# microsoft/Spartan2

Hardware: AMD Instinct MI355X
Metric: sha256_spartan prove(): R1CS constraints/sec (prove wall-clock in ms_per_step) (higher is better)
Workload: dtype u256 modular integer (8 x u32 Montgomery limbs; T256 scalar/base fields)

## Files before the change

### spartan2_amd/csrc/capi_core.hip

```cpp
#include <atomic>
#include <chrono>
#include <cstdlib>
#include <cstdio>
#include <cstring>

#include "core.hpp"
#include "walk_pool.hpp"
#include "kernels_poly.hpp"

namespace sp {
static thread_local std::string g_err;
static thread_local sp_wait_hook g_wait_hook = nullptr;
static thread_local void* g_wait_user = nullptr;
void set_error(const std::string& m) { g_err = m; }
static std::atomic<int> g_live_contexts{0};
int live_contexts() { return g_live_contexts.load(std::memory_order_relaxed); }
void relax() {
  if (g_wait_hook) g_wait_hook(g_wait_user);
  else __builtin_ia32_pause();
}
void slow_note(const char* site, long spins) {
  static const bool on = getenv("SPARTAN_SLOWPATH_LOG") != nullptr;
  if (on) fprintf(stderr, "[slow path] %s after %ld polls\n", site, spins);
}
// ... 546 lines not shown
}
static bool fold_stage2_enabled() {
  static const bool on = [] {
    const char* e = getenv("SPARTAN_FOLD_STAGE2");
    return e && e[0] == '1';
  }();
  return on;
}
static spk::LazyOut lazy_out(sp_ctx* c, spk::lazy9_t* lp, size_t nparts, int gl, const fe_t* eq_out, unsigned seq) {
  spk::LazyOut lo(lp);
  const size_t ngroups = nparts >> gl;
  size_t b2 = (ngroups + 63) / 64;
  if (b2 < 1) b2 = 1;
  if (b2 > (size_t)spk::HOST_SUM_MAX_BLOCKS) b2 = spk::HOST_SUM_MAX_BLOCKS;
  lo.eq_out = eq_out;
  lo.mapped = c->d_pinned;
  lo.seq = seq;
  lo.nslots = (unsigned)b2;
  lo.gl = gl;
  static const unsigned fold_slots = [] {
    const char* e = getenv("SPARTAN_FOLD_SLOTS");
    const int v = e ? atoi(e) : spk::HOST_SUM_MAX_BLOCKS;
    return (unsigned)(v < 1 ? 1 : (v > spk::HOST_SUM_MAX_BLOCKS ? spk::HOST_SUM_MAX_BLOCKS : v));
  }();
  size_t fs = fold_slots;
  while (fs > 1 && (fs > ngroups || ngroups % fs)) fs >>= 1;
  const bool even = ngroups > 0 && ((size_t)ngroups << gl) == nparts && ngroups % fs == 0 && (gl == 0 || nparts % 2 == 0);
  if (fold_stage2_enabled() && even && c->d_fold_tickets) {
    lo.tickets = c->d_fold_tickets;
    lo.nslots = (unsigned)fs;
    lo.per_slot = (unsigned)(nparts / fs);
  }
  return lo;
}
static void sum_lazy_launch(sp_ctx* c, const spk::LazyOut& lo, size_t nparts) {
  const int gl = lo.gl;
  const unsigned seq = lo.seq;
  const fe_t* eq_out = lo.eq_out;
  c->pending_slots = lo.nslots;
  if (lo.tickets) return;
  const uint32_t* P = reinterpret_cast<const uint32_t*>(lo.P);
  const dim3 g(lo.nslots), b(64);
  const bool vec_ok = nparts % 8 == 0;
  if (vec_ok && gl == 0) hipLaunchKernelGGL((spk::k_sum_partials_lazy<0>), g, b, 0, c->stream, P, nparts, gl, eq_out, c->d_pinned, seq);
  else if (vec_ok && gl == 1) hipLaunchKernelGGL((spk::k_sum_partials_lazy<1>), g, b, 0, c->stream, P, nparts, gl, eq_out, c->d_pinned, seq);
  else if (vec_ok && gl == 2) hipLaunchKernelGGL((spk::k_sum_partials_lazy<2>), g, b, 0, c->stream, P, nparts, gl, eq_out, c->d_pinned, seq);
  else if (vec_ok && gl == 3) hipLaunchKernelGGL((spk::k_sum_partials_lazy<3>), g, b, 0, c->stream, P, nparts, gl, eq_out, c->d_pinned, seq);
  else hipLaunchKernelGGL((spk::k_sum_partials_lazy<-1>), g, b, 0, c->stream, P, nparts, gl, eq_out, c->d_pinned, seq);
}
static int wait_slot(sp_ctx* c, const fe_t* slot, unsigned want, int nvals, fe_t* v, bool resident, long* spins) {
  volatile const unsigned* fl = reinterpret_cast<volatile const unsigned*>(slot + 3);
  while (*fl != want) {
    if (++*spins > 400000) {
      sp::slow_note("wait_slot", *spins);
      if (resident) {
        const auto t0 = std::chrono::steady_clock::now();
        while (*fl != want) {
          if (std::chrono::steady_clock::now() - t0 > std::chrono::seconds(12)) return fail(SP_ERR_INTERNAL, "sum-check tail kernel did not deliver a round result");
          sp::relax();
        }
        break;
      }
      SP_HIP(sp::stream_sync(c->stream));
      if (*fl != want) return fail(SP_ERR_INTERNAL, "evaluation kernel did not deliver its block sums");
    }
    sp::relax();
// ... 336 lines not shown
      c->h_mail[spk::MAIL_LINE_WORDS * l + 12] = v;
    }
    if (c->mail_dev) __builtin_ia32_sfence();
  };
  set_all(1);
  sp::stream_sync(c->stream);
  set_all(0);
  *reinterpret_cast<volatile uint32_t*>(c->h_pinned + spk::TAIL_ERR_ELEM) = 0;
}
struct AheadGuard {
  sp_ctx* c;
  bool armed = false;
  explicit AheadGuard(sp_ctx* ctx) : c(ctx) {}
  ~AheadGuard() {
    if (armed) tail_abort(c);
  }
};
static spk::MailRef mail_ref(sp_ctx* c, bool ahead, unsigned answers) {
  spk::MailRef m;
  m.mail = ahead ? c->d_mail : nullptr;
  m.mirror = c->d_mail_mirror;
  m.mapped = c->d_pinned;
  m.answers = answers;
  m.gated = nullptr;
  return m;
}
static spk::MailRef gate_launch(sp_ctx* c, unsigned answers) {
  fe_t* slot = c->d_gate + (answers & (spk::MAIL_RING - 1));
  hipLaunchKernelGGL(spk::k_mail_gate, dim3(1), dim3(64), 0, c->stream, mail_ref(c, true, answers), slot);
  spk::MailRef m = mail_ref(c, false, answers);
  m.gated = slot;
  return m;
}
static bool gate_ok(sp_ctx* c) {
  static const bool off = [] {
    const char* e = getenv("SPARTAN_GATE");
    return e && e[0] == '0';
  }();
  return c->mail_dev && !off;
}
static bool launch_ahead_ok(sp_ctx* c, size_t table_len) {
  return c->mail_dev && table_len <= ((size_t)1 << 19);
}
static unsigned tail_blocks(size_t len, bool cubic = false) {
  const size_t q = len / 2, wq = cubic ? spk::TAIL_WIDE_Q_CUBIC : spk::TAIL_WIDE_Q;
  if (q <= wq) return 1u;
  const size_t nb = q / wq;
  return (unsigned)(cubic && nb == 2 * (size_t)spk::HOST_SUM_MAX_BLOCKS ? nb / 2 : nb);
}
static std::atomic<int> g_tail_resident{0};
static int tail_block_budget() {
  static const int v = [] {
    const char* e = getenv("SPARTAN_TAIL_BUDGET");
    const int b = e ? atoi(e) : 64;
    return b < 0 ? 0 : b;
  }();
  return v;
}
struct TailLease {
  int n = 0;
  bool take(unsigned blocks) {
    if (blocks <= 1) return true;
    if (g_tail_resident.fetch_add((int)blocks) + (int)blocks > tail_block_budget()) {
      g_tail_resident.fetch_sub((int)blocks);
      return false;
    }
// ... 386 lines not shown
    eq_in = d_pr + spk::eq_level_offset((int)(ell - 1));
    sbits = 63;
    mode = 0;
  }
  const unsigned seq = next_seq(c);
  const dim3 g((unsigned)blocks), b(256);
  c->timed("eval_cubic", 128ull * half, [&] {
    if (mode == 0) hipLaunchKernelGGL((spk::k_eval_cubic<0, false, true>), g, b, 0, c->stream, A->d, B->d, (const fe_t*)nullptr, half, eq_in, eq_out, sbits, d_part, c->d_pinned, seq);
    else if (mode == 1) hipLaunchKernelGGL((spk::k_eval_cubic<1, false, true>), g, b, 0, c->stream, A->d, B->d, (const fe_t*)nullptr, half, eq_in, eq_out, sbits, d_part, c->d_pinned, seq);
    else hipLaunchKernelGGL((spk::k_eval_cubic<2, false, true>), g, b, 0, c->stream, A->d, B->d, (const fe_t*)nullptr, half, eq_in, eq_out, sbits, d_part, c->d_pinned, seq);
  });
  fe_t sums[2];
  if ((rc = reduce_partials(c, blocks, 2, sums))) return rc;
  const fe_t tinf = sums[1], one = fe_one<S>(), tau = taus[0];
  const fe_t eq0 = fe_sub<S>(one, tau), slope = fe_sub<S>(tau, eq0), eqm1 = fe_sub<S>(eq0, slope);
  const fe_t s_0 = fe_zero(), s_1 = fe_zero();
  const fe_t s_leading = fe_mul<S>(slope, tinf);
  const fe_t s_m1 = fe_mul<S>(eqm1, fe_dbl<S>(tinf));
  const fe_t halfc = two_inv();
  const fe_t c1 = fe_sub<S>(fe_mul<S>(fe_sub<S>(s_1, s_m1), halfc), s_leading);
  const fe_t c2 = fe_sub<S>(fe_mul<S>(fe_add<S>(s_1, s_m1), halfc), s_0);
  const fe_t inner_2 = fe_add<S>(c2, fe_dbl<S>(s_leading));
  const fe_t eval_2 = fe_add<S>(s_0, fe_dbl<S>(fe_add<S>(c1, fe_dbl<S>(inner_2))));
  const fe_t c3_3 = fe_add<S>(fe_dbl<S>(s_leading), s_leading);
  const fe_t inner_3 = fe_add<S>(c2, c3_3);
  const fe_t mid_3 = fe_add<S>(fe_add<S>(c1, fe_dbl<S>(inner_3)), inner_3);
  const fe_t eval_3 = fe_add<S>(fe_add<S>(s_0, fe_dbl<S>(mid_3)), mid_3);
  store_fe(out, s_0);
  store_fe(out + 4, eval_2);
  store_fe(out + 8, eval_3);
  return SP_OK;
}

static bool table_dense(const sp_table* t) { return sp::eff_lo(t) == t->len / 2 && sp::eff_hi(t) == t->len / 2; }

static int quad_impl(sp_ctx* c, uint64_t claim_io[4], size_t rounds, sp_table* A, sp_table* B, sp_transcript* tr, sp_reduce_hook reduce, void* reduce_user,
                     sp_challenge_hook observe, void* observe_user, uint64_t* out_cpolys, uint64_t* out_r, uint64_t out_final[8], size_t run_rounds = 0);
int sp_sumcheck_quad(sp_ctx* c, const uint64_t claim_[4], size_t rounds, sp_table* A, sp_table* B, sp_transcript* tr, uint64_t* out_cpolys,
                     uint64_t* out_r, uint64_t out_final[8]) {
  uint64_t claim_io[4];
  memcpy(claim_io, claim_, 32);
  return quad_impl(c, claim_io, rounds, A, B, tr, nullptr, nullptr, sp::pcs_ahead_wants(c, rounds) ? &sp::pcs_ahead_on_challenge : nullptr, c, out_cpolys, out_r, out_final);
}
int sp_sumcheck_quad_observed(sp_ctx* c, const uint64_t claim_[4], size_t rounds, sp_table* A, sp_table* B, sp_transcript* tr, sp_challenge_hook observe,
                              void* user, uint64_t* out_cpolys, uint64_t* out_r, uint64_t out_final[8]) {
  uint64_t claim_io[4];
  memcpy(claim_io, claim_, 32);
  return quad_impl(c, claim_io, rounds, A, B, tr, nullptr, nullptr, observe, user, out_cpolys, out_r, out_final);
}
int sp_sumcheck_quad_sharded(sp_ctx* c, uint64_t claim_io[4], size_t rounds, sp_table* A, sp_table* B, sp_transcript* tr, sp_reduce_hook reduce, void* reduce_user,
                             uint64_t* out_cpolys, uint64_t* out_r, uint64_t out_final[8]) {
  return quad_impl(c, claim_io, rounds, A, B, tr, reduce, reduce_user, nullptr, nullptr, out_cpolys, out_r, out_final);
}

int sp_sumcheck_quad_sharded_observed(sp_ctx* c, uint64_t claim_io[4], size_t rounds, sp_table* A, sp_table* B, sp_transcript* tr, sp_reduce_hook reduce,
                                      void* reduce_user, sp_challenge_hook observe, void* observe_user, uint64_t* out_cpolys, uint64_t* out_r, uint64_t out_final[8]) {
  return quad_impl(c, claim_io, rounds, A, B, tr, reduce, reduce_user, observe, observe_user, out_cpolys, out_r, out_final);
}

int sp_sumcheck_quad_sharded_partial(sp_ctx* c, uint64_t claim_io[4], size_t rounds, size_t run_rounds, sp_table* A, sp_table* B, sp_transcript* tr,
                                     sp_reduce_hook reduce, void* reduce_user, sp_challenge_hook observe, void* observe_user, uint64_t* out_cpolys, uint64_t* out_r) {
  if (run_rounds == 0 || run_rounds >= rounds) return fail(SP_ERR_INVALID_INPUT_LENGTH, "prove_quad (partial): 0 < run_rounds < rounds");
  uint64_t unused[8];
  return quad_impl(c, claim_io, rounds, A, B, tr, reduce, reduce_user, observe, observe_user, out_cpolys, out_r, unused, run_rounds);
}

// ... 97 lines not shown
      have_sums = true;
      return 1;
    }
    if (sparse_stream) {
      const size_t q = A->len / 4;
      const unsigned seq = next_seq(c);
      const spk::LazyOut lp = lazy_out(c, reinterpret_cast<spk::lazy9_t*>(c->d_scratch), q / 256, 2, nullptr, seq);
      c->timed("bind_stream_quad_sparse", 64ull * (A->len / 2) * 2, [&] {
        hipLaunchKernelGGL(spk::k_bind_eval_quad_stream_sparse, dim3((unsigned)(q / 256)), dim3(256), 0, c->stream, A->d, B->d, q, rv, sp::eff_hi(A), sp::eff_hi(B), lp,
                           mref);
      });
      sum_lazy_launch(c, lp, q / 256);
      sp::after_bind(A);
      sp::after_bind(B);
      have_sums = true;
      return 1;
    }
    if (ahead) return 0;
    sp_table* tabs[2] = {A, B};
    have_sums = false;
    int rc2 = launch_bind(c, tabs, 2, rv);
    return rc2 ? rc2 : 1;
  };
  for (size_t round = 0; round < rounds; ++round) {
    const size_t half = A->len / 2, len_now = A->len;
    const double tr0 = round_trace() ? now_us() : 0;
    fe_t sums[2] = {fe_zero(), fe_zero()};
    bool waiting = have_sums;
    if (!have_sums && !host_mode) {
      size_t len = sp::eff_pairs(A);
      if (sp::eff_pairs(B) < len) len = sp::eff_pairs(B);
      if (half < len) len = half;
      if (len >= STREAM_MIN_Q && len % 1024 == 0) {
        const unsigned seq = next_seq(c);
        const size_t hi_max = sp::eff_hi(A) > sp::eff_hi(B) ? sp::eff_hi(A) : sp::eff_hi(B);
        const bool lowhi = hi_max <= len / 2;
        const size_t blocks = len / (256 * (size_t)4);
        const spk::LazyOut lp = lazy_out(c, reinterpret_cast<spk::lazy9_t*>(c->d_scratch), blocks, 2, nullptr, seq);
        c->timed("eval_quad", 64ull * len + 32ull * ((sp::eff_hi(A) < len ? sp::eff_hi(A) : len) + (sp::eff_hi(B) < len ? sp::eff_hi(B) : len)), [&] {
          if (lowhi)
            hipLaunchKernelGGL((spk::k_eval_quad_stream_lowhi<4>), dim3((unsigned)blocks), dim3(256), 0, c->stream, A->d, B->d, half, sp::eff_hi(A), sp::eff_hi(B), lp);
          else
            hipLaunchKernelGGL((spk::k_eval_quad_stream<4>), dim3((unsigned)blocks), dim3(256), 0, c->stream, A->d, B->d, half, sp::eff_hi(A), sp::eff_hi(B), lp);
        });
        sum_lazy_launch(c, lp, blocks);
        waiting = true;
      } else if (len > 0) {
        size_t blocks = (len + chunk - 1) / chunk;
        c->timed("eval_quad", 64ull * len + 32ull * ((sp::eff_hi(A) < len ? sp::eff_hi(A) : len) + (sp::eff_hi(B) < len ? sp::eff_hi(B) : len)),
                 [&] { hipLaunchKernelGGL(spk::k_eval_quad, dim3((unsigned)blocks), dim3(256), 0, c->stream, A->d, B->d, half, len, sp::eff_hi(A), sp::eff_hi(B), c->d_scratch, c->d_pinned, next_seq(c)); });
        reduce_partials_launch(c, blocks, 2);
        waiting = true;
      }
    }
    const unsigned wait_seq = c->result_seq, wait_slots = c->pending_slots;
    const bool wait_resident = in_tail;
    if (wait_resident && !host_mode && spk::tail_hand_over(len_now, tail_hand_n(false))) {
      hA.resize(2 * len_now);
      if ((rc = wait_hand_over(c, wait_seq, (int)(2 * len_now), hA.data()))) return rc;
      hB = hA.data() + len_now;
      host_mode = true;
      hand_seq = wait_seq;
    }
    if (host_mode) {
      host_quad_eval(hA.data(), hB, half, sums);
      waiting = false;
    }
    if (!host_mode && wait_resident && spk::tail_double(false, len_now, tail_hand_n(false))) {
      fe_t S8[8];
// ... 1243 lines not shown
```

### spartan2_amd/csrc/kernels_poly.hpp

```cpp
#pragma once
#include "device_utils.hpp"

namespace spk {

constexpr int RESULT_FLAG_ELEM = 7;
__device__ __forceinline__ void publish_result(fe_t* result, unsigned seq) {
  __threadfence_system();
  __hip_atomic_store(reinterpret_cast<unsigned*>(result + RESULT_FLAG_ELEM), seq, __ATOMIC_RELEASE, __HIP_MEMORY_SCOPE_SYSTEM);
}

constexpr int HOST_SUM_MAX_BLOCKS = 64;
constexpr int SLOT_BASE_ELEM = 64;
struct slot_chk {
  unsigned a, b;
};
constexpr unsigned SLOT_CHK_K = 0x9E3779B1u;
__host__ __device__ __forceinline__ void slot_chk_add(slot_chk& c, const fe_t& v, int k) {
  unsigned plain = 0, ramp = 0;
#pragma unroll
  for (int i = 0; i < 8; ++i) {
    plain += v.v[i];
    ramp += (unsigned)i * v.v[i];
  }
  c.a += plain;
  c.b += (unsigned)(8 * k + 1) * plain + ramp;
}
__device__ __forceinline__ void slot_store_elem(fe_t* dst, const fe_t& v) { *dst = v; }
__device__ __forceinline__ void slot_store_tag(fe_t* slot, unsigned seq, const slot_chk& c) {
  const unsigned long long hi = ((unsigned long long)seq << 32) | (seq * SLOT_CHK_K + c.b);
  const unsigned long long lo = ((unsigned long long)(seq + c.a) << 32) | seq;
  __hip_atomic_store(reinterpret_cast<unsigned long long*>(&slot[3].v[2]), hi, __ATOMIC_RELAXED, __HIP_MEMORY_SCOPE_SYSTEM);
  __hip_atomic_store(reinterpret_cast<unsigned long long*>(&slot[3].v[0]), lo, __ATOMIC_RELAXED, __HIP_MEMORY_SCOPE_SYSTEM);
}
template <int NACC>
// ... 141 lines not shown
      if (lane == 0) {
        unsigned* e = reinterpret_cast<unsigned*>(mapped + TAIL_ERR_ELEM);
        e[1] = want;
        e[2] = blockIdx.x;
        e[3] = gridDim.x;
        __hip_atomic_store(e, 1u, __ATOMIC_RELEASE, __HIP_MEMORY_SCOPE_SYSTEM);
      }
    }
    if (lane == 0) ok = good;
  }
  __syncthreads();
  return ok != 0;
}
__device__ __forceinline__ fe_t gated_challenge(const fe_t* p) {
  typedef const __attribute__((address_space(4))) uint32_t* const_words;
  const_words q = (const_words)(uintptr_t)p;
  fe_t r;
#pragma unroll
  for (int i = 0; i < 8; ++i) r.v[i] = q[i];
  return r;
}
__device__ __forceinline__ fe_t challenge_or(const MailRef& m, const fe_t& r_arg) {
  if (m.gated) return gated_challenge(m.gated);
  if (!m.mail) return r_arg;
  __shared__ fe_t r_sh;
  mail_wait(m.mail, m.mirror, m.mapped, m.answers, &r_sh);
  return r_sh;
}

__global__ void __launch_bounds__(64) k_mail_gate(MailRef m, fe_t* __restrict__ out) {
  __shared__ fe_t r_sh;
  mail_wait(m.mail, m.mirror, m.mapped, m.answers, &r_sh);
  if (threadIdx.x < 8) out->v[threadIdx.x] = r_sh.v[threadIdx.x];
}

constexpr int BIND_MAX_TABLES = 8;
struct BindArgs {
  fe_t* z[BIND_MAX_TABLES];
  unsigned long long n[BIND_MAX_TABLES];
  unsigned long long lo[BIND_MAX_TABLES];
  unsigned long long hi[BIND_MAX_TABLES];
  fe_t r;
  fe_t one_minus_r;
};
__global__ void __launch_bounds__(256) k_bind_top(BindArgs a) {
  const int t = blockIdx.y;
  fe_t* __restrict__ Z = a.z[t];
  const unsigned long long n = a.n[t], lo = a.lo[t], hi = a.hi[t];
  const unsigned long long eff = lo > hi ? lo : hi;
  const unsigned long long both = lo < hi ? lo : hi;
  for (unsigned long long i = (unsigned long long)blockIdx.x * blockDim.x + threadIdx.x; i < eff; i += (unsigned long long)gridDim.x * blockDim.x) {
    fe_t out;
    if (i < both) {
      fe_t lo_v = Z[i], hi_v = Z[n + i];
      out = fe_add<S>(lo_v, fe_mul<S>(a.r, fe_sub<S>(hi_v, lo_v)));
    } else if (i < lo) {
      out = fe_mul<S>(Z[i], a.one_minus_r);
    } else {
      out = fe_mul<S>(a.r, Z[n + i]);
    }
    Z[i] = out;
  }
}

__host__ __device__ __forceinline__ size_t eq_level_offset(int k) { return ((size_t)1 << k) - 1; }
constexpr int EQ_LDS_ENTRIES = 1024;
// ... 158 lines not shown
      const fe_t eo = eq_out[base >> s];
      acc[0] = fe_mul<S>(acc[0], eo);
      acc[1] = fe_mul<S>(acc[1], eo);
    }
    emit_partials<2>(acc, partials, single_out, seq);
  }
}
__global__ void __launch_bounds__(256) k_bind_eval_quad(fe_t* __restrict__ A, fe_t* __restrict__ B, size_t q, fe_t r_arg, fe_t* __restrict__ partials,
                                                        fe_t* __restrict__ single_out, unsigned seq, MailRef mref) {
  __shared__ fe_t smem[2 * 4];
  const size_t id = (size_t)blockIdx.x * blockDim.x + threadIdx.x;
  const bool live = id < q;
  const size_t ld = live ? id : 0;
  const fe_t la0 = A[ld], la1 = A[ld + q], la2 = A[ld + 2 * q], la3 = A[ld + 3 * q];
  const fe_t lb0 = B[ld], lb1 = B[ld + q], lb2 = B[ld + 2 * q], lb3 = B[ld + 3 * q];
  const fe_t r = challenge_or(mref, r_arg);
  fe_t acc[2] = {fe_zero(), fe_zero()};
  if (live) {
    const fe_t a0 = bind1(la0, la2, r), a1 = bind1(la1, la3, r);
    const fe_t b0 = bind1(lb0, lb2, r), b1 = bind1(lb1, lb3, r);
    A[id] = a0;
    A[id + q] = a1;
    B[id] = b0;
    B[id + q] = b1;
    acc[0] = fe_mul<S>(a0, b0);
    acc[1] = fe_mul<S>(fe_sub<S>(a1, a0), fe_sub<S>(b1, b0));
  }
  block_sum<2>(acc, smem);
  if (threadIdx.x == 0) {
    emit_partials<2>(acc, partials, single_out, seq);
  }
}

template <bool AGENT>
__device__ __forceinline__ void lazy_slot_sums(const uint32_t* __restrict__ P, size_t nparts, int gl, const fe_t* __restrict__ eq_out, fe_t* __restrict__ mapped, unsigned seq,
                                               unsigned slot, unsigned nslots, int lane) {
  const size_t ngroups = nparts >> gl, per = (size_t)1 << gl;
  fe_t acc[2] = {fe_zero(), fe_zero()};
  const size_t G = ngroups / nslots;
  for (size_t g = (size_t)slot * G + lane; g < (size_t)(slot + 1) * G; g += 64) {
    fe_t f[2];
#pragma unroll
    for (int a = 0; a < 2; ++a) {
      lazy9_t l;
      unsigned long long carry = 0;
#pragma unroll
      for (int w = 0; w < 9; ++w) {
        const uint32_t* src = P + (size_t)(2 * w + a) * nparts + g * per;
        unsigned long long t = carry;
        if (per == 1) {
          t += AGENT ? __hip_atomic_load(src, __ATOMIC_RELAXED, __HIP_MEMORY_SCOPE_AGENT) : src[0];
        } else {
          const unsigned long long* s2 = reinterpret_cast<const unsigned long long*>(src);
          for (size_t k = 0; k < per / 2; ++k) {
            const unsigned long long v = AGENT ? __hip_atomic_load(s2 + k, __ATOMIC_RELAXED, __HIP_MEMORY_SCOPE_AGENT) : s2[k];
            t += (v & 0xffffffffull) + (v >> 32);
          }
        }
        l.v[w] = (uint32_t)t;
        carry = t >> 32;
      }
      f[a] = lazy_reduce(l);
    }
    if (eq_out) {
      const fe_t eo = eq_out[g];
      f[0] = fe_mul<S>(f[0], eo);
      f[1] = fe_mul<S>(f[1], eo);
    }
    acc[0] = fe_add<S>(acc[0], f[0]);
    acc[1] = fe_add<S>(acc[1], f[1]);
  }
  acc[0] = wave_sum(acc[0]);
  acc[1] = wave_sum(acc[1]);
  if (lane == 0) {
    fe_t* sl = mapped + SLOT_BASE_ELEM + 4 * slot;
    slot_chk chk = {0u, 0u};
#pragma unroll
    for (int k = 0; k < 2; ++k) {
      slot_store_elem(sl + k, acc[k]);
      slot_chk_add(chk, acc[k], k);
    }
    slot_store_tag(sl, seq, chk);
  }
}
__device__ __forceinline__ void stream_block_partials(const lazy9_t& s0, const lazy9_t& s1, LazyOut partials) {
  __shared__ lazy9_t sm[4][2];
  __shared__ unsigned last_sh;
  const int lane = threadIdx.x & 63, wave = threadIdx.x >> 6;
  if (lane == 0) {
    sm[wave][0] = s0;
    sm[wave][1] = s1;
  }
  __syncthreads();
  const bool fold = partials.tickets != nullptr;
  if (threadIdx.x < 2) {
    const lazy9_t t = lazy_add(lazy_add(sm[0][threadIdx.x], sm[1][threadIdx.x]), lazy_add(sm[2][threadIdx.x], sm[3][threadIdx.x]));
    uint32_t* P = reinterpret_cast<uint32_t*>(partials.P);
    if (fold) {
#pragma unroll
      for (int w = 0; w < 9; ++w) __hip_atomic_store(P + (size_t)(2 * w + threadIdx.x) * gridDim.x + blockIdx.x, t.v[w], __ATOMIC_RELAXED, __HIP_MEMORY_SCOPE_AGENT);
      asm volatile("s_waitcnt vmcnt(0)" ::: "memory");
    } else {
#pragma unroll
      for (int w = 0; w < 9; ++w) P[(size_t)(2 * w + threadIdx.x) * gridDim.x + blockIdx.x] = t.v[w];
    }
  }
  if (!fold) return;
  __syncthreads();
  if (threadIdx.x == 0) {
    const unsigned slot = (unsigned)(blockIdx.x / partials.per_slot);
    const unsigned old = __hip_atomic_fetch_add(partials.tickets + slot, 1u, __ATOMIC_RELAXED, __HIP_MEMORY_SCOPE_AGENT);
    last_sh = old + 1 == partials.per_slot ? slot + 1 : 0u;
  }
  __syncthreads();
  if (last_sh == 0 || threadIdx.x >= 64) return;
  const unsigned slot = last_sh - 1;
  if (threadIdx.x == 0) __hip_atomic_store(partials.tickets + slot, 0u, __ATOMIC_RELAXED, __HIP_MEMORY_SCOPE_AGENT);
  lazy_slot_sums<true>(reinterpret_cast<const uint32_t*>(partials.P), gridDim.x, partials.gl, partials.eq_out, partials.mapped, partials.seq, slot, partials.nslots, lane);
}
template <int MODE, bool AHEAD, bool GATED = false>
__global__ void __launch_bounds__(256) k_bind_eval_cubic_stream(fe_t* __restrict__ A, fe_t* __restrict__ B, fe_t* __restrict__ C, size_t q, fe_t r_arg,
                                                                const fe_t* __restrict__ eq_in, int s, LazyOut partials, MailRef mref) {
  const size_t id = (size_t)blockIdx.x * blockDim.x + threadIdx.x;
  const size_t mask = ((size_t)1 << s) - 1;
  const fe_t la0 = A[id], la1 = A[id + q], la2 = A[id + 2 * q], la3 = A[id + 3 * q];
  const fe_t lb0 = B[id], lb1 = B[id + q], lb2 = B[id + 2 * q], lb3 = B[id + 3 * q];
  const fe_t lc0 = C[id], lc1 = C[id + q], lc2 = C[id + 2 * q], lc3 = C[id + 3 * q];
  fe_t r = r_arg;
  if (AHEAD) r = challenge_or(mref, r_arg);
  if (GATED) r = gated_challenge(mref.gated);
  const fe_t a0 = bind1(la0, la2, r), a1 = bind1(la1, la3, r);
  const fe_t b0 = bind1(lb0, lb2, r), b1 = bind1(lb1, lb3, r);
  const fe_t c0 = bind1(lc0, lc2, r), c1 = bind1(lc1, lc3, r);
  A[id] = a0;
  A[id + q] = a1;
  B[id] = b0;
  B[id + q] = b1;
  C[id] = c0;
  C[id + q] = c1;
  const fe_t w = (MODE == 0) ? eq_in[id] : eq_in[id & mask];
  const fe_t t0e = fe_sub<S>(fe_mul<S>(a0, b0), c0);
  const fe_t tie = fe_mul<S>(fe_sub<S>(a1, a0), fe_sub<S>(b1, b0));
  stream_block_partials(lazy_wave_sum(lazy_from(fe_mul<S>(w, t0e))), lazy_wave_sum(lazy_from(fe_mul<S>(w, tie))), partials);
}
template <int MODE>
__global__ void __launch_bounds__(256) k_eval_cubic_stream(const fe_t* __restrict__ A, const fe_t* __restrict__ B, const fe_t* __restrict__ C, size_t half,
                                                           const fe_t* __restrict__ eq_in, int s, LazyOut partials) {
  const size_t id = (size_t)blockIdx.x * blockDim.x + threadIdx.x;
  const size_t mask = ((size_t)1 << s) - 1;
  const fe_t a0 = A[id], a1 = A[id + half], b0 = B[id], b1 = B[id + half], c0 = C[id];
  const fe_t w = (MODE == 0) ? eq_in[id] : eq_in[id & mask];
// ... 27 lines not shown
    l0 = lazy_wave_sum(l0);
  }
  stream_block_partials(l0, l1, partials);
}
__global__ void __launch_bounds__(256) k_bind_eval_quad_stream(fe_t* __restrict__ A, fe_t* __restrict__ B, size_t q, fe_t r_arg, LazyOut partials,
                                                               MailRef mref) {
  const size_t id = (size_t)blockIdx.x * blockDim.x + threadIdx.x;
  const fe_t la0 = A[id], la1 = A[id + q], la2 = A[id + 2 * q], la3 = A[id + 3 * q];
  const fe_t lb0 = B[id], lb1 = B[id + q], lb2 = B[id + 2 * q], lb3 = B[id + 3 * q];
  const fe_t r = challenge_or(mref, r_arg);
  const fe_t a0 = bind1(la0, la2, r), a1 = bind1(la1, la3, r);
  const fe_t b0 = bind1(lb0, lb2, r), b1 = bind1(lb1, lb3, r);
  A[id] = a0;
  A[id + q] = a1;
  B[id] = b0;
  B[id + q] = b1;
  stream_block_partials(lazy_wave_sum(lazy_from(fe_mul<S>(a0, b0))), lazy_wave_sum(lazy_from(fe_mul<S>(fe_sub<S>(a1, a0), fe_sub<S>(b1, b0)))), partials);
}
__global__ void __launch_bounds__(256) k_bind_eval_quad_stream_sparse(fe_t* __restrict__ A, fe_t* __restrict__ B, size_t q, fe_t r_arg, size_t hiA, size_t hiB,
                                                                      LazyOut partials, MailRef mref) {
  const size_t id = (size_t)blockIdx.x * blockDim.x + threadIdx.x;
  const fe_t la0 = A[id], la1 = A[id + q], lb0 = B[id], lb1 = B[id + q];
  const fe_t r = challenge_or(mref, r_arg);
  const fe_t one_minus_r = fe_sub<S>(fe_one<S>(), r);
  const fe_t a0 = id < hiA ? bind1(la0, A[id + 2 * q], r) : fe_mul<S>(la0, one_minus_r);
  const fe_t b0 = id < hiB ? bind1(lb0, B[id + 2 * q], r) : fe_mul<S>(lb0, one_minus_r);
  const fe_t a1 = fe_mul<S>(la1, one_minus_r), b1 = fe_mul<S>(lb1, one_minus_r);
  A[id] = a0;
  A[id + q] = a1;
  B[id] = b0;
  B[id + q] = b1;
  stream_block_partials(lazy_wave_sum(lazy_from(fe_mul<S>(a0, b0))), lazy_wave_sum(lazy_from(fe_mul<S>(fe_sub<S>(a1, a0), fe_sub<S>(b1, b0)))), partials);
}
template <int PPT>
__global__ void __launch_bounds__(256) k_eval_quad_stream(const fe_t* __restrict__ A, const fe_t* __restrict__ B, size_t half, size_t hiA, size_t hiB,
                                                          LazyOut partials) {
  const size_t stride = (size_t)gridDim.x * blockDim.x;
  size_t id = (size_t)blockIdx.x * blockDim.x + threadIdx.x;
  lazy9_t l0 = lazy_from(fe_zero()), l1 = lazy_from(fe_zero());
#pragma unroll
  for (int k = 0; k < PPT; ++k, id += stride) {
    const fe_t a0 = A[id], b0 = B[id];
    const fe_t a1 = id < hiA ? A[id + half] : fe_zero(), b1 = id < hiB ? B[id + half] : fe_zero();
    l0 = lazy_add(l0, lazy_from(fe_mul<S>(a0, b0)));
    l1 = lazy_add(l1, lazy_from(fe_mul<S>(fe_sub<S>(a1, a0), fe_sub<S>(b1, b0))));
  }
  stream_block_partials(lazy_wave_sum(l0), lazy_wave_sum(l1), partials);
}
template <int PPT>
__global__ void __launch_bounds__(256) k_eval_quad_stream_lowhi(const fe_t* __restrict__ A, const fe_t* __restrict__ B, size_t half, size_t hiA, size_t hiB,
                                                                LazyOut partials) {
  const size_t stride = (size_t)gridDim.x * blockDim.x;
  const size_t id0 = (size_t)blockIdx.x * blockDim.x + threadIdx.x;
  fe_t a0[PPT], b0[PPT];
#pragma unroll
  for (int k = 0; k < PPT; ++k) {
    a0[k] = A[id0 + k * stride];
    b0[k] = B[id0 + k * stride];
  }
  lazy9_t l0 = lazy_from(fe_zero()), l1 = lazy_from(fe_zero());
#pragma unroll
  for (int k = 0; k < PPT; ++k) {
    const size_t id = id0 + k * stride;
    const fe_t p = fe_mul<S>(a0[k], b0[k]);
    l0 = lazy_add(l0, lazy_from(p));
    if (id < hiA || id < hiB) {
      const fe_t a1 = id < hiA ? A[id + half] : fe_zero(), b1 = id < hiB ? B[id + half] : fe_zero();
      l1 = lazy_add(l1, lazy_from(fe_sub<S>(fe_mul<S>(fe_sub<S>(a1, a0[k]), fe_sub<S>(b1, b0[k])), p)));
    }
  }
  l1 = lazy_add(l1, l0);
  stream_block_partials(lazy_wave_sum(l0), lazy_wave_sum(l1), partials);
}
template <int GL>
__global__ void __launch_bounds__(64) k_sum_partials_lazy(const uint32_t* __restrict__ P, size_t nparts, int gl_rt, const fe_t* __restrict__ eq_out,
                                                          fe_t* __restrict__ mapped, unsigned seq) {
  const int gl = GL >= 0 ? GL : gl_rt;
  const size_t ngroups = nparts >> gl, per = (size_t)1 << gl;
  fe_t acc[2] = {fe_zero(), fe_zero()};
  for (size_t g = (size_t)blockIdx.x * 64 + threadIdx.x; g < ngroups; g += (size_t)gridDim.x * 64) {
    unsigned long long col[2][9];
#pragma unroll
    for (int w = 0; w < 9; ++w)
#pragma unroll
      for (int a = 0; a < 2; ++a) {
        const uint32_t* src = P + (size_t)(2 * w + a) * nparts + g * per;
        if constexpr (GL == 0) {
          col[a][w] = src[0];
        } else if constexpr (GL == 1) {
          const uint2 v = *reinterpret_cast<const uint2*>(src);
          col[a][w] = (unsigned long long)v.x + v.y;
        } else if constexpr (GL == 2) {
          const uint4 v = *reinterpret_cast<const uint4*>(src);
          col[a][w] = ((unsigned long long)v.x + v.y) + ((unsigned long long)v.z + v.w);
        } else if constexpr (GL == 3) {
          const uint4 v = *reinterpret_cast<const uint4*>(src), u = *reinterpret_cast<const uint4*>(src + 4);
          col[a][w] = (((unsigned long long)v.x + v.y) + ((unsigned long long)v.z + v.w)) + (((unsigned long long)u.x + u.y) + ((unsigned long long)u.z + u.w));
        } else {
          unsigned long long t = 0;
          for (size_t k = 0; k < per; ++k) t += src[k];
          col[a][w] = t;
        }
      }
    fe_t f[2];
#pragma unroll
    for (int a = 0; a < 2; ++a) {
      lazy9_t l;
      unsigned long long carry = 0;
#pragma unroll
      for (int w = 0; w < 9; ++w) {
        const unsigned long long t = col[a][w] + carry;
        l.v[w] = (uint32_t)t;
        carry = t >> 32;
      }
      f[a] = lazy_reduce(l);
    }
    if (eq_out) {
      const fe_t eo = eq_out[g];
      f[0] = fe_mul<S>(f[0], eo);
      f[1] = fe_mul<S>(f[1], eo);
    }
    acc[0] = fe_add<S>(acc[0], f[0]);
    acc[1] = fe_add<S>(acc[1], f[1]);
  }
  acc[0] = wave_sum(acc[0]);
  acc[1] = wave_sum(acc[1]);
  if (threadIdx.x == 0) emit_partials<2>(acc, nullptr, mapped, seq);
}

__global__ void __launch_bounds__(256) k_eval_quad(const fe_t* __restrict__ A, const fe_t* __restrict__ B, size_t half, size_t len, size_t hiA, size_t hiB,
                                                   fe_t* __restrict__ partials, fe_t* __restrict__ single_out, unsigned seq) {
  __shared__ fe_t smem[2 * 4];
  const size_t chunk = (size_t)blockDim.x * EVAL_PPT;
  const size_t base = (size_t)blockIdx.x * chunk;
  fe_t acc[2] = {fe_zero(), fe_zero()};
#pragma unroll 1
  for (int k = 0; k < EVAL_PPT; ++k) {
    const size_t id = base + (size_t)k * blockDim.x + threadIdx.x;
    if (id < len) {
      const fe_t a0 = A[id], b0 = B[id];
      const fe_t a1 = id < hiA ? A[id + half] : fe_zero(), b1 = id < hiB ? B[id + half] : fe_zero();
      acc[0] = fe_add<S>(acc[0], fe_mul<S>(a0, b0));
      acc[1] = fe_add<S>(acc[1], fe_mul<S>(fe_sub<S>(a1, a0), fe_sub<S>(b1, b0)));
    }
  }
  block_sum<2>(acc, smem);
  if (threadIdx.x == 0) {
    emit_partials<2>(acc, partials, single_out, seq);
  }
}

template <bool FALLBACK>
__global__ void __launch_bounds__(256) k_eval_cubic_outer_pow(const fe_t* __restrict__ pleft, size_t left, const fe_t* __restrict__ pright, size_t right,
                                                              const fe_t* __restrict__ A, const fe_t* __restrict__ B, const fe_t* __restrict__ C, size_t len,
                                                              fe_t* __restrict__ partials, fe_t* __restrict__ single_out, unsigned seq) {
  __shared__ fe_t smem[3 * 4];
  fe_t acc[3] = {fe_zero(), fe_zero(), fe_zero()};
  const size_t low = (size_t)blockIdx.x * blockDim.x + threadIdx.x;
  if (low < len) {
    fe_t tl, th;
// ... 576 lines not shown
```

Measured before the change: 1.042 billion.

## Carry two quad sumcheck rounds per device pass using sparse-tail algebra

Adds a fast path to the quadratic sumcheck for sparse-tail tables: one kernel computes three partial sums (low, high, cross) plus head terms for the sparse upper part. The host then derives both the round-0 and round-1 polynomials from these sums in closed form. Bind and evaluation for the two challenges are fused into one carry kernel, gated on both challenges through a two-slot mail gate. This removes one full eval pass, one bind pass and one host-device round trip per pair of rounds, at the cost of more complex algebra and new generalized NS-way partial reduction code.

```diff
diff --git a/spartan2_amd/csrc/capi_core.hip b/spartan2_amd/csrc/capi_core.hip
--- a/spartan2_amd/csrc/capi_core.hip
+++ b/spartan2_amd/csrc/capi_core.hip
@@ -602,6 +602,14 @@
     lo.per_slot = (unsigned)(nparts / fs);
   }
   return lo;
+}
+static void sum_lazy_launch3(sp_ctx* c, const spk::LazyOut& lo, size_t nparts) {
+  c->pending_slots = lo.nslots;
+  if (lo.tickets) return;
+  const uint32_t* P = reinterpret_cast<const uint32_t*>(lo.P);
+  const dim3 g(lo.nslots), b(64);
+  if (nparts % 8 == 0 && lo.gl == 2) hipLaunchKernelGGL((spk::k_sum_partials_lazy<2, 3>), g, b, 0, c->stream, P, nparts, lo.gl, lo.eq_out, c->d_pinned, lo.seq);
+  else hipLaunchKernelGGL((spk::k_sum_partials_lazy<-1, 3>), g, b, 0, c->stream, P, nparts, lo.gl, lo.eq_out, c->d_pinned, lo.seq);
 }
 static void sum_lazy_launch(sp_ctx* c, const spk::LazyOut& lo, size_t nparts) {
   const int gl = lo.gl;
@@ -1004,6 +1012,9 @@
   m.gated = slot;
   return m;
 }
+static void gate2_launch(sp_ctx* c, unsigned answers) {
+  hipLaunchKernelGGL(spk::k_mail_gate2, dim3(1), dim3(64), 0, c->stream, mail_ref(c, true, answers), c->d_gate);
+}
 static bool gate_ok(sp_ctx* c) {
   static const bool off = [] {
     const char* e = getenv("SPARTAN_GATE");
@@ -1456,6 +1467,9 @@
   return SP_OK;
 }
 
+static const size_t QUAD_CARRY_MAX_HI = 1024;
+static void spk_quad_carry_round0(const quad_carry_sums& q, fe_t& s0, fe_t& s2) { quad_carry_round0<S>(q, s0, s2); }
+static void spk_quad_carry_round1(const quad_carry_sums& q, const fe_t& r0, fe_t& s0, fe_t& s2) { quad_carry_round1<S>(q, r0, s0, s2); }
 static bool table_dense(const sp_table* t) { return sp::eff_lo(t) == t->len / 2 && sp::eff_hi(t) == t->len / 2; }
 
 static int quad_impl(sp_ctx* c, uint64_t claim_io[4], size_t rounds, sp_table* A, sp_table* B, sp_transcript* tr, sp_reduce_hook reduce, void* reduce_user,
@@ -1619,9 +1633,100 @@
       if (sp::eff_pairs(B) < len) len = sp::eff_pairs(B);
       if (half < len) len = half;
       if (len >= STREAM_MIN_Q && len % 1024 == 0) {
-        const unsigned seq = next_seq(c);
         const size_t hi_max = sp::eff_hi(A) > sp::eff_hi(B) ? sp::eff_hi(A) : sp::eff_hi(B);
         const bool lowhi = hi_max <= len / 2;
+        const bool carry = lowhi && !reduce && !stopped && round + 2 < rounds && len == half && A->len / 4 >= STREAM_MIN_Q && sp::eff_lo(A) == half && sp::eff_lo(B) == half &&
+                           hi_max <= QUAD_CARRY_MAX_HI && hi_max <= A->len / 8 && (A->len / 8) % 256 == 0;
+        if (carry) {
+          const size_t hiA = sp::eff_hi(A), hiB = sp::eff_hi(B), h = half / 2, q = A->len / 8;
+          const unsigned head_blocks = (unsigned)((hi_max + 255) / 256);
+          const unsigned seq0 = next_seq(c);
+          const size_t blocks = h / 512;
+          const spk::LazyOut lp = lazy_out(c, reinterpret_cast<spk::lazy9_t*>(c->d_scratch), blocks, 2, nullptr, seq0);
+          c->timed("eval_quad", 64ull * half + 32ull * (hiA + hiB), [&] {
+            hipLaunchKernelGGL(spk::k_eval_quad_stream_two, dim3((unsigned)blocks), dim3(256), 0, c->stream, A->d, B->d, half, hiA, hiB, head_blocks, lp, c->d_pinned, seq0);
+          });
+          sum_lazy_launch3(c, lp, blocks);
+          const unsigned l_slots = c->pending_slots;
+          const unsigned seq1 = next_seq(c), seq2 = next_seq(c);
+          const spk::LazyOut bp = lazy_out(c, reinterpret_cast<spk::lazy9_t*>(c->d_scratch), q / 256, 2, nullptr, seq2);
+          auto launch_bind2 = [&](const fe_t& r0v, const fe_t& r1v, bool gated) {
+            c->timed("bind_stream_quad", 48ull * A->len, [&] {
+              hipLaunchKernelGGL(spk::k_bind_eval_quad_stream_carry, dim3((unsigned)(q / 256)), dim3(256), 0, c->stream, A->d, B->d, q, r0v, r1v, hiA, hiB, bp,
+                                 gated ? c->d_gate + (seq0 & (spk::MAIL_RING - 1)) : nullptr, gated ? c->d_gate + (seq1 & (spk::MAIL_RING - 1)) : nullptr);
+            });
+            sum_lazy_launch(c, bp, q / 256);
+          };
+          const bool ahead2 = c->mail_dev && gate_ok(c);
+          if (ahead2) {
+            gate2_launch(c, seq0);
+            launch_bind2(fe_zero(), fe_zero(), true);
+            guard.armed = true;
+          }
+          const unsigned bind_slots = bp.nslots;
+          quad_carry_sums cs;
+          fe_t three[3];
+          c->result_seq = seq0;
+          c->pending_slots = l_slots;
+          if ((rc = reduce_partials_wait(c, 3, three, ahead2))) return rc;
+          cs.L_lo = three[0];
+          cs.L_hi = three[1];
+          cs.L_x = three[2];
+          three[0] = three[1] = three[2] = fe_zero();
+          if (head_blocks) {
+            c->result_seq = seq0;
+            c->pending_slots = head_blocks;
+            if ((rc = reduce_partials_wait(c, 3, three, ahead2, 1, true))) return rc;
+          }
+          cs.X1 = three[0];
+          cs.X2 = three[1];
+          cs.Y1 = three[2];
+          c->result_seq = seq2;
+          fe_t rr[2];
+          double t_prev = tr0;
+          for (int k = 0; k < 2; ++k) {
+            const double t_wait = round_trace() ? now_us() : 0;
+            fe_t e0, tinf;
+            if (k == 0) spk_quad_carry_round0(cs, e0, tinf);
+            else spk_quad_carry_round1(cs, rr[0], e0, tinf);
+            UniPoly poly;
+            poly.n = 3;
+            poly.c[0] = e0;
+            poly.c[1] = fe_sub<S>(fe_sub<S>(claim, fe_dbl<S>(e0)), tinf);
+            poly.c[2] = tinf;
+            absorb_poly(tr->t, poly);
+            if (!tr->t.squeeze<S>(lbl_c, 1, &rr[k])) return fail(SP_ERR_INTERNAL_TRANSCRIPT, "transcript round counter overflow");
+            if (ahead2) tail_post_challenge(c, rr[k], k == 0 ? seq0 : seq1);
+            else if (k == 1) launch_bind2(rr[0], rr[1], false);
+            store_fe(out_r + 4 * (round + k), rr[k]);
+            store_fe(out_cpolys + 8 * (round + k), poly.c[0]);
+            store_fe(out_cpolys + 8 * (round + k) + 4, poly.c[2]);
+            claim = poly_eval(poly, rr[k]);
+            if (observe) {
+              uint64_t rw[4];
+              store_fe(rw, rr[k]);
+              observe(observe_user, round + k, rw);
+            }
+            if (round_trace()) {
+              const double t_end = now_us();
+              fprintf(stderr, "quad round %2zu len %8zu tail 0 wait %7.1f us host %6.1f us%s\n", round + k, k == 0 ? len_now : len_now / 2, k == 0 ? t_wait - t_prev : 0.0,
+                      t_end - t_wait, k == 0 ? "" : " (host only: first bind carried)");
+              t_prev = t_end;
+            }
+          }
+          for (int k = 0; k < 2; ++k) {
+            sp::after_bind(A);
+            sp::after_bind(B);
+          }
+          c->result_seq = seq2;
+          c->pending_slots = bind_slots;
+          have_sums = true;
+          last_answered = seq1;
+          guard.armed = false;
+          ++round;
+          continue;
+        }
+        const unsigned seq = next_seq(c);
         const size_t blocks = len / (256 * (size_t)4);
         const spk::LazyOut lp = lazy_out(c, reinterpret_cast<spk::lazy9_t*>(c->d_scratch), blocks, 2, nullptr, seq);
         c->timed("eval_quad", 64ull * len + 32ull * ((sp::eff_hi(A) < len ? sp::eff_hi(A) : len) + (sp::eff_hi(B) < len ? sp::eff_hi(B) : len)), [&] {
diff --git a/spartan2_amd/csrc/kernels_poly.hpp b/spartan2_amd/csrc/kernels_poly.hpp
--- a/spartan2_amd/csrc/kernels_poly.hpp
+++ b/spartan2_amd/csrc/kernels_poly.hpp
@@ -1,5 +1,6 @@
 #pragma once
 #include "device_utils.hpp"
+#include "quad_carry.hpp"
 
 namespace spk {
 
@@ -207,6 +208,17 @@
   __shared__ fe_t r_sh;
   mail_wait(m.mail, m.mirror, m.mapped, m.answers, &r_sh);
   if (threadIdx.x < 8) out->v[threadIdx.x] = r_sh.v[threadIdx.x];
+}
+
+__global__ void __launch_bounds__(64) k_mail_gate2(MailRef m, fe_t* __restrict__ out) {
+  __shared__ fe_t r_sh;
+#pragma unroll 1
+  for (unsigned k = 0; k < 2; ++k) {
+    const unsigned want = m.answers + k;
+    mail_wait(m.mail, m.mirror, m.mapped, want, &r_sh);
+    if (threadIdx.x < 8) out[want & (MAIL_RING - 1)].v[threadIdx.x] = r_sh.v[threadIdx.x];
+    __syncthreads();
+  }
 }
 
 constexpr int BIND_MAX_TABLES = 8;
@@ -431,21 +443,23 @@
   }
 }
 
-template <bool AGENT>
+template <bool AGENT, int NS = 2>
 __device__ __forceinline__ void lazy_slot_sums(const uint32_t* __restrict__ P, size_t nparts, int gl, const fe_t* __restrict__ eq_out, fe_t* __restrict__ mapped, unsigned seq,
                                                unsigned slot, unsigned nslots, int lane) {
   const size_t ngroups = nparts >> gl, per = (size_t)1 << gl;
-  fe_t acc[2] = {fe_zero(), fe_zero()};
+  fe_t acc[NS];
+#pragma unroll
+  for (int a = 0; a < NS; ++a) acc[a] = fe_zero();
   const size_t G = ngroups / nslots;
   for (size_t g = (size_t)slot * G + lane; g < (size_t)(slot + 1) * G; g += 64) {
-    fe_t f[2];
-#pragma unroll
-    for (int a = 0; a < 2; ++a) {
+    fe_t f[NS];
+#pragma unroll
+    for (int a = 0; a < NS; ++a) {
       lazy9_t l;
       unsigned long long carry = 0;
 #pragma unroll
       for (int w = 0; w < 9; ++w) {
-        const uint32_t* src = P + (size_t)(2 * w + a) * nparts + g * per;
+        const uint32_t* src = P + (size_t)(NS * w + a) * nparts + g * per;
         unsigned long long t = carry;
         if (per == 1) {
           t += AGENT ? __hip_atomic_load(src, __ATOMIC_RELAXED, __HIP_MEMORY_SCOPE_AGENT) : src[0];
@@ -463,45 +477,46 @@
     }
     if (eq_out) {
       const fe_t eo = eq_out[g];
-      f[0] = fe_mul<S>(f[0], eo);
-      f[1] = fe_mul<S>(f[1], eo);
-    }
-    acc[0] = fe_add<S>(acc[0], f[0]);
-    acc[1] = fe_add<S>(acc[1], f[1]);
-  }
-  acc[0] = wave_sum(acc[0]);
-  acc[1] = wave_sum(acc[1]);
+#pragma unroll
+      for (int a = 0; a < NS; ++a) f[a] = fe_mul<S>(f[a], eo);
+    }
+#pragma unroll
+    for (int a = 0; a < NS; ++a) acc[a] = fe_add<S>(acc[a], f[a]);
+  }
+#pragma unroll
+  for (int a = 0; a < NS; ++a) acc[a] = wave_sum(acc[a]);
   if (lane == 0) {
     fe_t* sl = mapped + SLOT_BASE_ELEM + 4 * slot;
     slot_chk chk = {0u, 0u};
 #pragma unroll
-    for (int k = 0; k < 2; ++k) {
+    for (int k = 0; k < NS; ++k) {
       slot_store_elem(sl + k, acc[k]);
       slot_chk_add(chk, acc[k], k);
     }
     slot_store_tag(sl, seq, chk);
   }
 }
-__device__ __forceinline__ void stream_block_partials(const lazy9_t& s0, const lazy9_t& s1, LazyOut partials) {
-  __shared__ lazy9_t sm[4][2];
+template <int NS>
+__device__ __forceinline__ void stream_block_partials_n(const lazy9_t (&s)[NS], LazyOut partials) {
+  __shared__ lazy9_t sm[4][NS];
   __shared__ unsigned last_sh;
   const int lane = threadIdx.x & 63, wave = threadIdx.x >> 6;
   if (lane == 0) {
-    sm[wave][0] = s0;
-    sm[wave][1] = s1;
+#pragma unroll
+    for (int a = 0; a < NS; ++a) sm[wave][a] = s[a];
   }
   __syncthreads();
   const bool fold = partials.tickets != nullptr;
-  if (threadIdx.x < 2) {
+  if (threadIdx.x < NS) {
     const lazy9_t t = lazy_add(lazy_add(sm[0][threadIdx.x], sm[1][threadIdx.x]), lazy_add(sm[2][threadIdx.x], sm[3][threadIdx.x]));
     uint32_t* P = reinterpret_cast<uint32_t*>(partials.P);
     if (fold) {
 #pragma unroll
-      for (int w = 0; w < 9; ++w) __hip_atomic_store(P + (size_t)(2 * w + threadIdx.x) * gridDim.x + blockIdx.x, t.v[w], __ATOMIC_RELAXED, __HIP_MEMORY_SCOPE_AGENT);
+      for (int w = 0; w < 9; ++w) __hip_atomic_store(P + (size_t)(NS * w + threadIdx.x) * gridDim.x + blockIdx.x, t.v[w], __ATOMIC_RELAXED, __HIP_MEMORY_SCOPE_AGENT);
       asm volatile("s_waitcnt vmcnt(0)" ::: "memory");
     } else {
 #pragma unroll
-      for (int w = 0; w < 9; ++w) P[(size_t)(2 * w + threadIdx.x) * gridDim.x + blockIdx.x] = t.v[w];
+      for (int w = 0; w < 9; ++w) P[(size_t)(NS * w + threadIdx.x) * gridDim.x + blockIdx.x] = t.v[w];
     }
   }
   if (!fold) return;
@@ -515,7 +530,11 @@
   if (last_sh == 0 || threadIdx.x >= 64) return;
   const unsigned slot = last_sh - 1;
   if (threadIdx.x == 0) __hip_atomic_store(partials.tickets + slot, 0u, __ATOMIC_RELAXED, __HIP_MEMORY_SCOPE_AGENT);
-  lazy_slot_sums<true>(reinterpret_cast<const uint32_t*>(partials.P), gridDim.x, partials.gl, partials.eq_out, partials.mapped, partials.seq, slot, partials.nslots, lane);
+  lazy_slot_sums<true, NS>(reinterpret_cast<const uint32_t*>(partials.P), gridDim.x, partials.gl, partials.eq_out, partials.mapped, partials.seq, slot, partials.nslots, lane);
+}
+__device__ __forceinline__ void stream_block_partials(const lazy9_t& s0, const lazy9_t& s1, LazyOut partials) {
+  const lazy9_t s[2] = {s0, s1};
+  stream_block_partials_n<2>(s, partials);
 }
 template <int MODE, bool AHEAD, bool GATED = false>
 __global__ void __launch_bounds__(256) k_bind_eval_cubic_stream(fe_t* __restrict__ A, fe_t* __restrict__ B, fe_t* __restrict__ C, size_t q, fe_t r_arg,
@@ -609,6 +628,27 @@
   B[id + q] = b1;
   stream_block_partials(lazy_wave_sum(lazy_from(fe_mul<S>(a0, b0))), lazy_wave_sum(lazy_from(fe_mul<S>(fe_sub<S>(a1, a0), fe_sub<S>(b1, b0)))), partials);
 }
+__global__ void __launch_bounds__(256) k_bind_eval_quad_stream_carry(fe_t* __restrict__ A, fe_t* __restrict__ B, size_t q, fe_t r0_arg, fe_t r1_arg, size_t hiA, size_t hiB,
+                                                                     LazyOut partials, const fe_t* __restrict__ gated0, const fe_t* __restrict__ gated1) {
+  const size_t id = (size_t)blockIdx.x * blockDim.x + threadIdx.x;
+  const fe_t la0 = A[id], la1 = A[id + q], la2 = A[id + 2 * q], la3 = A[id + 3 * q];
+  const fe_t lb0 = B[id], lb1 = B[id + q], lb2 = B[id + 2 * q], lb3 = B[id + 3 * q];
+  const fe_t r0 = gated0 ? gated_challenge(gated0) : r0_arg, r1 = gated1 ? gated_challenge(gated1) : r1_arg;
+  const fe_t c = fe_sub<S>(fe_one<S>(), r0);
+  fe_t a0 = fe_mul<S>(c, bind1(la0, la2, r1)), a1 = fe_mul<S>(c, bind1(la1, la3, r1));
+  fe_t b0 = fe_mul<S>(c, bind1(lb0, lb2, r1)), b1 = fe_mul<S>(c, bind1(lb1, lb3, r1));
+  if (id < hiA || id < hiB) {
+    fe_t alpha, beta, gamma;
+    quad_carry_bind_coeffs<S>(r0, r1, alpha, beta, gamma);
+    if (id < hiA) a0 = fe_add<S>(a0, fe_mul<S>(gamma, A[id + 4 * q]));
+    if (id < hiB) b0 = fe_add<S>(b0, fe_mul<S>(gamma, B[id + 4 * q]));
+  }
+  A[id] = a0;
+  A[id + q] = a1;
+  B[id] = b0;
+  B[id + q] = b1;
+  stream_block_partials(lazy_wave_sum(lazy_from(fe_mul<S>(a0, b0))), lazy_wave_sum(lazy_from(fe_mul<S>(fe_sub<S>(a1, a0), fe_sub<S>(b1, b0)))), partials);
+}
 template <int PPT>
 __global__ void __launch_bounds__(256) k_eval_quad_stream(const fe_t* __restrict__ A, const fe_t* __restrict__ B, size_t half, size_t hiA, size_t hiB,
                                                           LazyOut partials) {
@@ -649,19 +689,58 @@
   l1 = lazy_add(l1, l0);
   stream_block_partials(lazy_wave_sum(l0), lazy_wave_sum(l1), partials);
 }
-template <int GL>
+__global__ void __launch_bounds__(256, 4) k_eval_quad_stream_two(const fe_t* __restrict__ A, const fe_t* __restrict__ B, size_t half, size_t hiA, size_t hiB, unsigned head_blocks,
+                                                              LazyOut partials, fe_t* __restrict__ mapped, unsigned seq) {
+  const size_t h = half / 2, stride = (size_t)gridDim.x * blockDim.x;
+  const size_t id0 = (size_t)blockIdx.x * blockDim.x + threadIdx.x;
+  fe_t al[2], ah[2], bl[2], bh[2];
+#pragma unroll
+  for (int k = 0; k < 2; ++k) {
+    al[k] = A[id0 + k * stride];
+    ah[k] = A[id0 + k * stride + h];
+    bl[k] = B[id0 + k * stride];
+    bh[k] = B[id0 + k * stride + h];
+  }
+  lazy9_t l[3] = {lazy_from(fe_zero()), lazy_from(fe_zero()), lazy_from(fe_zero())};
+#pragma unroll
+  for (int k = 0; k < 2; ++k) {
+    l[0] = lazy_add(l[0], lazy_from(fe_mul<S>(al[k], bl[k])));
+    l[1] = lazy_add(l[1], lazy_from(fe_mul<S>(ah[k], bh[k])));
+    l[2] = lazy_add(l[2], lazy_from(fe_mul<S>(fe_sub<S>(ah[k], al[k]), fe_sub<S>(bh[k], bl[k]))));
+  }
+#pragma unroll
+  for (int a = 0; a < 3; ++a) l[a] = lazy_wave_sum(l[a]);
+  stream_block_partials_n<3>(l, partials);
+  if (blockIdx.x < head_blocks) {
+    __shared__ fe_t head_sm[3 * 4];
+    fe_t x[3] = {fe_zero(), fe_zero(), fe_zero()};
+    if (id0 < hiA || id0 < hiB) {
+      const fe_t aH = id0 < hiA ? A[id0 + half] : fe_zero(), bH = id0 < hiB ? B[id0 + half] : fe_zero();
+      const fe_t a0 = A[id0], b0 = B[id0];
+      const fe_t da = fe_sub<S>(A[id0 + h], a0), db = fe_sub<S>(B[id0 + h], b0);
+      x[0] = fe_add<S>(fe_mul<S>(a0, bH), fe_mul<S>(aH, b0));
+      x[1] = fe_mul<S>(aH, bH);
+      x[2] = fe_add<S>(fe_mul<S>(da, bH), fe_mul<S>(aH, db));
+    }
+    block_sum<3>(x, head_sm);
+    if (threadIdx.x == 0) emit_partials_wide<3>(x, mapped, seq);
+  }
+}
+template <int GL, int NS = 2>
 __global__ void __launch_bounds__(64) k_sum_partials_lazy(const uint32_t* __restrict__ P, size_t nparts, int gl_rt, const fe_t* __restrict__ eq_out,
                                                           fe_t* __restrict__ mapped, unsigned seq) {
   const int gl = GL >= 0 ? GL : gl_rt;
   const size_t ngroups = nparts >> gl, per = (size_t)1 << gl;
-  fe_t acc[2] = {fe_zero(), fe_zero()};
+  fe_t acc[NS];
+#pragma unroll
+  for (int a = 0; a < NS; ++a) acc[a] = fe_zero();
   for (size_t g = (size_t)blockIdx.x * 64 + threadIdx.x; g < ngroups; g += (size_t)gridDim.x * 64) {
-    unsigned long long col[2][9];
+    unsigned long long col[NS][9];
 #pragma unroll
     for (int w = 0; w < 9; ++w)
 #pragma unroll
-      for (int a = 0; a < 2; ++a) {
-        const uint32_t* src = P + (size_t)(2 * w + a) * nparts + g * per;
+      for (int a = 0; a < NS; ++a) {
+        const uint32_t* src = P + (size_t)(NS * w + a) * nparts + g * per;
         if constexpr (GL == 0) {
           col[a][w] = src[0];
         } else if constexpr (GL == 1) {
@@ -679,9 +758,9 @@
           col[a][w] = t;
         }
       }
-    fe_t f[2];
-#pragma unroll
-    for (int a = 0; a < 2; ++a) {
+    fe_t f[NS];
+#pragma unroll
+    for (int a = 0; a < NS; ++a) {
       lazy9_t l;
       unsigned long long carry = 0;
 #pragma unroll
@@ -694,15 +773,15 @@
     }
     if (eq_out) {
       const fe_t eo = eq_out[g];
-      f[0] = fe_mul<S>(f[0], eo);
-      f[1] = fe_mul<S>(f[1], eo);
-    }
-    acc[0] = fe_add<S>(acc[0], f[0]);
-    acc[1] = fe_add<S>(acc[1], f[1]);
-  }
-  acc[0] = wave_sum(acc[0]);
-  acc[1] = wave_sum(acc[1]);
-  if (threadIdx.x == 0) emit_partials<2>(acc, nullptr, mapped, seq);
+#pragma unroll
+      for (int a = 0; a < NS; ++a) f[a] = fe_mul<S>(f[a], eo);
+    }
+#pragma unroll
+    for (int a = 0; a < NS; ++a) acc[a] = fe_add<S>(acc[a], f[a]);
+  }
+#pragma unroll
+  for (int a = 0; a < NS; ++a) acc[a] = wave_sum(acc[a]);
+  if (threadIdx.x == 0) emit_partials<NS>(acc, nullptr, mapped, seq);
 }
 
 __global__ void __launch_bounds__(256) k_eval_quad(const fe_t* __restrict__ A, const fe_t* __restrict__ B, size_t half, size_t len, size_t hiA, size_t hiB,
diff --git a/spartan2_amd/csrc/quad_carry.hpp b/spartan2_amd/csrc/quad_carry.hpp
--- /dev/null
+++ b/spartan2_amd/csrc/quad_carry.hpp
@@ -0,0 +1,25 @@
+#pragma once
+#include "field.hpp"
+
+struct quad_carry_sums {
+  fe_t L_lo, L_hi, L_x, X1, X2, Y1;
+};
+template <class FP>
+SP_HD void quad_carry_round0(const quad_carry_sums& q, fe_t& s0, fe_t& s2) {
+  s0 = fe_add<FP>(q.L_lo, q.L_hi);
+  s2 = fe_add<FP>(fe_sub<FP>(s0, q.X1), q.X2);
+}
+template <class FP>
+SP_HD void quad_carry_round1(const quad_carry_sums& q, const fe_t& r0, fe_t& s0, fe_t& s2) {
+  const fe_t c = fe_sub<FP>(fe_one<FP>(), r0);
+  const fe_t cc = fe_mul<FP>(c, c), cr = fe_mul<FP>(c, r0), rrx2 = fe_mul<FP>(fe_mul<FP>(r0, r0), q.X2);
+  s0 = fe_add<FP>(fe_add<FP>(fe_mul<FP>(cc, q.L_lo), fe_mul<FP>(cr, q.X1)), rrx2);
+  s2 = fe_add<FP>(fe_sub<FP>(fe_mul<FP>(cc, q.L_x), fe_mul<FP>(cr, q.Y1)), rrx2);
+}
+template <class FP>
+SP_HD void quad_carry_bind_coeffs(const fe_t& r0, const fe_t& r1, fe_t& alpha, fe_t& beta, fe_t& gamma) {
+  const fe_t c = fe_sub<FP>(fe_one<FP>(), r0);
+  beta = fe_mul<FP>(c, r1);
+  alpha = fe_sub<FP>(c, beta);
+  gamma = fe_sub<FP>(r0, fe_mul<FP>(r1, r0));
+}
```

After: 1.041 billion. About the same (-0.1%).
